# filrg/split_learning

Hardware: AMD Instinct MI355X
Metric: images/sec (whole node) VGG16/CIFAR10 cut=7 (higher is better)
Workload: dtype fp32; 1 GPU; model=VGG16_CIFAR10, global_batch=32, image=3x32x32, cut_layer=7, optimizer=SGD(lr=5e-4, momentum=0.5), control_count=1, mode=serial-recompute, parallelism=split2 x dp1

## Files before the change

### split_learning_amd/ops/build.py

```python

from __future__ import annotations

import os
import subprocess
import sys
import sysconfig
from concurrent.futures import ThreadPoolExecutor

HERE = os.path.dirname(os.path.abspath(__file__))
CSRC = os.path.join(HERE, "csrc")
OUT_SO = os.path.join(HERE, "_sl_kernels.so")
BUILD_DIR = os.path.join(HERE, "_build")

SOURCES = [
    "gemm_f32.hip",
    "conv2d.hip",
    "wino.hip",
    "norm.hip",
    "elementwise.hip",
    "loss.hip",
    "attention.hip",
    "optim.hip",
    "bindings.cpp",
]

ARCH = os.environ.get("PYTORCH_ROCM_ARCH", "gfx950")


def _flags():
    import torch
    import torch.utils.cpp_extension as cpp_ext

    torch_lib = os.path.join(os.path.dirname(torch.__file__), "lib")
    includes = cpp_ext.include_paths(device_type="cuda")
    includes.append(sysconfig.get_paths()["include"])
    abi = int(getattr(torch._C, "_GLIBCXX_USE_CXX11_ABI", True))
    cxxflags = [
        "-O3", "-std=c++17", "-fPIC",
        f"--offload-arch={ARCH}",
        f"-D_GLIBCXX_USE_CXX11_ABI={abi}",
        "-DTORCH_EXTENSION_NAME=_sl_kernels",
        "-DTORCH_API_INCLUDE_EXTENSION_H",
        "-DUSE_ROCM=1",
        "-D__HIP_PLATFORM_AMD__=1",
        "-DHIP_ENABLE_WARP_SYNC_BUILTINS=1",
        "-Wno-deprecated-declarations",
        "-fno-gpu-rdc",
    ] + [f"-I{p}" for p in includes]
    if os.environ.get("SLK_MFMA32"):
        cxxflags.append("-DSLK_MFMA32")
    ldflags = [
        "-shared",
        f"-L{torch_lib}", "-ltorch", "-ltorch_cpu", "-ltorch_python", "-lc10",
        "-ltorch_hip", "-lc10_hip",
        "-L/opt/rocm/lib", "-lamdhip64",
        f"-Wl,-rpath,{torch_lib}",
    ]
    return cxxflags, ldflags


def _run(cmd):
    proc = subprocess.run(cmd, capture_output=True, text=True)
    if proc.returncode != 0:
        raise RuntimeError(
            f"command failed ({proc.returncode}): {' '.join(cmd)}\n"
            f"stdout:\n{proc.stdout[-4000:]}\nstderr:\n{proc.stderr[-8000:]}")
    return proc


def build(verbose: bool = True, force: bool = False) -> str:
    os.makedirs(BUILD_DIR, exist_ok=True)
    hipcc = os.environ.get("HIPCC", "/opt/rocm/bin/hipcc")
    cxxflags, ldflags = _flags()

    objs = []
    jobs = []
    for src in SOURCES:
        sp = os.path.join(CSRC, src)
        op = os.path.join(BUILD_DIR, src.replace("/", "_") + ".o")
        objs.append(op)
        deps = [sp] + [os.path.join(CSRC, h) for h in (
            "common.h", "tile_gemm.h", "torch_util.h", "conv_route.h")]
        if (not force and os.path.exists(op)
                and all(os.path.getmtime(op) >= os.path.getmtime(d) for d in deps)):
            continue
        cmd = [hipcc, "-c", sp, "-o", op] + cxxflags
        if src.endswith(".cpp"):
            cmd.append("-x")
            cmd.append("c++")
        jobs.append(cmd)

    if jobs:
        if verbose:
            print(f"[build] compiling {len(jobs)} TU(s) with {hipcc} for {ARCH}")
        with ThreadPoolExecutor(max_workers=min(8, len(jobs))) as ex:
            list(ex.map(_run, jobs))

    if force or not os.path.exists(OUT_SO) or any(
            os.path.getmtime(o) > os.path.getmtime(OUT_SO) for o in objs):
        if verbose:
# ... 9 lines not shown
```

### split_learning_amd/ops/csrc/bindings.cpp

```cpp
#include <torch/extension.h>

namespace slk {
at::Tensor matmul_f32(const at::Tensor&, const at::Tensor&, bool, bool,
                      c10::optional<at::Tensor>, bool);
at::Tensor linear_fwd(const at::Tensor&, const at::Tensor&, c10::optional<at::Tensor>);
at::Tensor colsum_f32(const at::Tensor&);
at::Tensor conv2d_wino(const at::Tensor&, const at::Tensor&,
                       c10::optional<at::Tensor>, int, bool);
at::Tensor conv2d_wino_bwdw(const at::Tensor&, const at::Tensor&, int);
at::Tensor conv2d_wino_fused(const at::Tensor&, const at::Tensor&,
                             c10::optional<at::Tensor>, int, bool);
at::Tensor conv2d_wino_bwdw_fused(const at::Tensor&, const at::Tensor&, int);
at::Tensor conv2d_fwd(const at::Tensor&, const at::Tensor&, c10::optional<at::Tensor>,
                      int, int);
at::Tensor conv2d_bwd_data(const at::Tensor&, const at::Tensor&, int, int, int, int);
at::Tensor conv2d_bwd_weight(const at::Tensor&, const at::Tensor&, int, int, int, int);
at::Tensor conv2d_bwd_bias(const at::Tensor&);
std::string conv_route(const std::string&, int, int, int, int, int, int, int, int);
std::vector<at::Tensor> bn2d_stats_fused(const at::Tensor&,
                                         c10::optional<at::Tensor>,
                                         c10::optional<at::Tensor>,
                                         c10::optional<at::Tensor>, double, double);
at::Tensor bn2d_fwd(const at::Tensor&, const at::Tensor&, const at::Tensor&,
                    const at::Tensor&, const at::Tensor&, bool);
std::vector<at::Tensor> bn2d_bwd(const at::Tensor&, const at::Tensor&,
                                 const at::Tensor&, const at::Tensor&,
                                 const at::Tensor&, c10::optional<at::Tensor>);
std::vector<at::Tensor> bn2d_bwd_eval(const at::Tensor&, const at::Tensor&,
                                      const at::Tensor&, const at::Tensor&,
                                      const at::Tensor&, c10::optional<at::Tensor>);
std::vector<at::Tensor> bn2d_train_fwd(const at::Tensor&, const at::Tensor&,
                                       const at::Tensor&,
                                       c10::optional<at::Tensor>,
                                       c10::optional<at::Tensor>,
                                       c10::optional<at::Tensor>, double, double,
                                       bool, bool);
std::vector<at::Tensor> bn2d_train_bwd(const at::Tensor&, const at::Tensor&,
                                       const at::Tensor&, const at::Tensor&,
                                       const at::Tensor&, c10::optional<at::Tensor>,
                                       c10::optional<at::Tensor>);
std::vector<at::Tensor> drop_res_ln_fwd(const at::Tensor&, const at::Tensor&,
                                        const at::Tensor&, const at::Tensor&,
                                        double, double, int64_t,
                                        c10::optional<at::Tensor>);
std::vector<at::Tensor> layernorm_fwd(const at::Tensor&, const at::Tensor&,
                                      const at::Tensor&, double);
std::vector<at::Tensor> layernorm_bwd(const at::Tensor&, const at::Tensor&,
                                      const at::Tensor&, const at::Tensor&,
                                      const at::Tensor&);
at::Tensor relu_fwd(const at::Tensor&);
at::Tensor relu_bwd(const at::Tensor&, const at::Tensor&);
at::Tensor gelu_fwd(const at::Tensor&);
at::Tensor gelu_bwd(const at::Tensor&, const at::Tensor&);
at::Tensor tanh_fwd(const at::Tensor&);
at::Tensor tanh_bwd(const at::Tensor&, const at::Tensor&);
std::vector<at::Tensor> dropout_fwd(const at::Tensor&, double, int64_t, int64_t);
std::vector<at::Tensor> dropout_fwd_dev(const at::Tensor&, double, int64_t,
                                        const at::Tensor&);
at::Tensor dropout_bwd(const at::Tensor&, const at::Tensor&, double);
std::vector<at::Tensor> maxpool2x2_fwd(const at::Tensor&);
at::Tensor maxpool2x2_bwd(const at::Tensor&, const at::Tensor&, int, int);
at::Tensor embedding_fwd(const at::Tensor&, const at::Tensor&);
at::Tensor embedding_bwd(const at::Tensor&, const at::Tensor&, int64_t, int64_t);
std::vector<at::Tensor> attn_fwd(const at::Tensor&, const at::Tensor&,
                                 const at::Tensor&, double, double, int64_t,
                                 c10::optional<at::Tensor>);
at::Tensor softmax_fwd(const at::Tensor&);
at::Tensor softmax_bwd(const at::Tensor&, const at::Tensor&);
std::vector<at::Tensor> ce_fwd(const at::Tensor&, const at::Tensor&);
at::Tensor ce_bwd(const at::Tensor&, const at::Tensor&, const at::Tensor&);
void sgd_step(std::vector<at::Tensor>, std::vector<at::Tensor>,
              std::vector<at::Tensor>, double, double, double, bool, bool);
void adamw_step(std::vector<at::Tensor>, std::vector<at::Tensor>,
                std::vector<at::Tensor>, std::vector<at::Tensor>, int64_t, double,
                double, double, double, double, bool);
at::Tensor make_opt_desc(std::vector<at::Tensor>, std::vector<at::Tensor>,
                         std::vector<at::Tensor>, std::vector<at::Tensor>);
void sgd_step_fused(const at::Tensor&, int64_t, int64_t, double, double, double,
                    bool, bool);
void adamw_step_fused(const at::Tensor&, int64_t, int64_t, int64_t, double, double,
                      double, double, double, bool);
}

PYBIND11_MODULE(TORCH_EXTENSION_NAME, m) {
  m.doc() = "split_learning_amd CDNA4 (gfx950) HIP kernels";
  m.def("matmul_f32", &slk::matmul_f32, py::arg("a"), py::arg("b"),
        py::arg("trans_a") = false, py::arg("trans_b") = false,
        py::arg("out") = py::none(), py::arg("accumulate") = false);
  m.def("linear_fwd", &slk::linear_fwd);
  m.def("colsum_f32", &slk::colsum_f32);
  m.def("conv2d_wino", &slk::conv2d_wino, py::arg("x"), py::arg("w"),
        py::arg("bias") = py::none(), py::arg("pad") = 1,
        py::arg("flip") = false);
  m.def("conv2d_wino_bwdw", &slk::conv2d_wino_bwdw, py::arg("gy"),
        py::arg("x"), py::arg("pad") = 1);
  m.def("conv2d_wino_fused", &slk::conv2d_wino_fused, py::arg("x"),
        py::arg("w"), py::arg("bias") = py::none(), py::arg("pad") = 1,
        py::arg("flip") = false);
  m.def("conv2d_wino_bwdw_fused", &slk::conv2d_wino_bwdw_fused, py::arg("gy"),
        py::arg("x"), py::arg("pad") = 1);
  m.def("conv2d_fwd", &slk::conv2d_fwd, py::arg("x"), py::arg("w"),
        py::arg("bias"), py::arg("stride"), py::arg("pad"));
  m.def("conv2d_bwd_data", &slk::conv2d_bwd_data);
  m.def("conv2d_bwd_weight", &slk::conv2d_bwd_weight, py::arg("gy"), py::arg("x"),
        py::arg("kh"), py::arg("kw"), py::arg("stride"), py::arg("pad"));
  m.def("conv2d_bwd_bias", &slk::conv2d_bwd_bias);
  m.def("conv_route", &slk::conv_route, py::arg("op"), py::arg("B"),
        py::arg("Ci"), py::arg("H"), py::arg("W"), py::arg("Co"), py::arg("K"),
        py::arg("stride"), py::arg("pad"));
  m.def("bn2d_stats_fused", &slk::bn2d_stats_fused);
  m.def("bn2d_fwd", &slk::bn2d_fwd);
  m.def("bn2d_bwd", &slk::bn2d_bwd, py::arg("x"), py::arg("gy"),
        py::arg("gamma"), py::arg("mean"), py::arg("invstd"),
        py::arg("relu_y") = py::none());
  m.def("bn2d_bwd_eval", &slk::bn2d_bwd_eval, py::arg("x"), py::arg("gy"),
        py::arg("gamma"), py::arg("mean"), py::arg("invstd"),
        py::arg("relu_y") = py::none());
  m.def("bn2d_train_fwd", &slk::bn2d_train_fwd, py::arg("x"), py::arg("gamma"),
        py::arg("beta"), py::arg("running_mean"), py::arg("running_var"),
        py::arg("num_batches_tracked"), py::arg("momentum"), py::arg("eps"),
        py::arg("relu") = false, py::arg("pool") = false);
  m.def("bn2d_train_bwd", &slk::bn2d_train_bwd, py::arg("x"), py::arg("gy"),
        py::arg("gamma"), py::arg("mean"), py::arg("invstd"),
        py::arg("relu_y") = py::none(), py::arg("idx") = py::none());
  m.def("drop_res_ln_fwd", &slk::drop_res_ln_fwd, py::arg("x"), py::arg("res"),
        py::arg("gamma"), py::arg("beta"), py::arg("eps"), py::arg("p") = 0.0,
        py::arg("seed") = 0, py::arg("offset") = py::none());
  m.def("layernorm_fwd", &slk::layernorm_fwd);
  m.def("layernorm_bwd", &slk::layernorm_bwd);
  m.def("relu_fwd", &slk::relu_fwd);
  m.def("relu_bwd", &slk::relu_bwd);
  m.def("gelu_fwd", &slk::gelu_fwd);
  m.def("gelu_bwd", &slk::gelu_bwd);
  m.def("tanh_fwd", &slk::tanh_fwd);
  m.def("tanh_bwd", &slk::tanh_bwd);
  m.def("dropout_fwd", &slk::dropout_fwd);
  m.def("dropout_fwd_dev", &slk::dropout_fwd_dev);
  m.def("dropout_bwd", &slk::dropout_bwd);
  m.def("maxpool2x2_fwd", &slk::maxpool2x2_fwd);
  m.def("maxpool2x2_bwd", &slk::maxpool2x2_bwd);
  m.def("embedding_fwd", &slk::embedding_fwd);
  m.def("embedding_bwd", &slk::embedding_bwd);
  m.def("attn_fwd", &slk::attn_fwd, py::arg("q"), py::arg("k"), py::arg("v"),
        py::arg("scale"), py::arg("p") = 0.0, py::arg("seed") = 0,
        py::arg("offset") = py::none());
  m.def("softmax_fwd", &slk::softmax_fwd);
  m.def("softmax_bwd", &slk::softmax_bwd);
  m.def("ce_fwd", &slk::ce_fwd);
  m.def("ce_bwd", &slk::ce_bwd);
  m.def("sgd_step", &slk::sgd_step);
  m.def("adamw_step", &slk::adamw_step);
  m.def("make_opt_desc", &slk::make_opt_desc);
  m.def("sgd_step_fused", &slk::sgd_step_fused);
  m.def("adamw_step_fused", &slk::adamw_step_fused);
}
```

### split_learning_amd/ops/csrc/conv2d.hip

```cpp
#include <tuple>

#include "conv_route.h"
#include "tile_gemm.h"
#include "torch_util.h"

namespace slk {

at::Tensor conv2d_wino(const at::Tensor&, const at::Tensor&,
                       c10::optional<at::Tensor>, int, bool);
at::Tensor conv2d_wino_bwdw(const at::Tensor&, const at::Tensor&, int);
at::Tensor conv2d_wino_fused(const at::Tensor&, const at::Tensor&,
                             c10::optional<at::Tensor>, int, bool);
at::Tensor conv2d_wino_bwdw_fused(const at::Tensor&, const at::Tensor&, int);

static int wino_level() {
  static const int v = [] {
    const char* e = std::getenv("SLK_WINO");
    return e ? atoi(e) : 1;
  }();
  return v;
}

struct ConvGeom {
  int B, Ci, H, W, Co, KH, KW, OH, OW, stride, pad;
  FastDiv d_ohow, d_ow, d_hw, d_w, d_khkw, d_kw;
};

template <int CKH, int CKW, int CS>
struct Geo {
  static constexpr bool fixed = CKH > 0;
  __device__ static int kh_kw(const ConvGeom& g) { return fixed ? CKH * CKW : g.KH * g.KW; }
  __device__ static int stride(const ConvGeom& g) { return fixed ? CS : g.stride; }
  __device__ static void dk(const ConvGeom& g, int k, int& c, int& kh, int& kw) {
    if (fixed) {
      c = k / (CKH * CKW);
      const int r = k - c * (CKH * CKW);
      kh = r / CKW;
      kw = r - kh * CKW;
    } else {
      c = g.d_khkw.div(k);
      const int r = g.d_khkw.mod(k, c);
      kh = g.d_kw.div(r);
      kw = g.d_kw.mod(r, kh);
    }
  }
};

__device__ __forceinline__ float sel0(float v, bool keep) { return keep ? v : 0.f; }

template <int CKH, int CKW, int CS>
struct ConvFwdGather {
  using G = Geo<CKH, CKW, CS>;
  const float* w;
  const float* x;
  ConvGeom geo;

  struct KCtx {};
  __device__ KCtx prepK(int) const { return {}; }

  struct ACtx { int off; bool valid; };
  struct BCtx { int boff, ihb, iwb; bool valid; };

  __device__ ACtx prepA(int, int m, bool valid, int) const {
    return {(int)((long)m * (geo.Ci * G::kh_kw(geo))), valid};
  }
  __device__ float loadA(const ACtx& c, const KCtx&, int k, bool kv) const {
    return sel0(w[c.off + k], c.valid & kv);
  }
  __device__ BCtx prepB(int, int n, bool valid, int) const {
    const unsigned b = geo.d_ohow.div(n);
    const unsigned rem = geo.d_ohow.mod(n, b);
    const unsigned oh = geo.d_ow.div(rem);
    const unsigned ow = geo.d_ow.mod(rem, oh);
    return {(int)((long)b * geo.Ci * geo.H * geo.W),
            (int)oh * G::stride(geo) - geo.pad,
            (int)ow * G::stride(geo) - geo.pad, valid};
  }
  __device__ float loadB(const BCtx& c, const KCtx&, int k, bool kv) const {
    int ci, kh, kw;
    G::dk(geo, k, ci, kh, kw);
    const int ih = c.ihb + kh;
    const int iw = c.iwb + kw;
    const bool in = (unsigned)ih < (unsigned)geo.H && (unsigned)iw < (unsigned)geo.W;
    const int ihc = in ? ih : 0;
    const int iwc = in ? iw : 0;
    const float v = x[c.boff + (ci * geo.H + ihc) * geo.W + iwc];
    return sel0(v, c.valid & kv & in);
  }
};

struct ConvFwdStore {
  float* y;
// ... 300 lines not shown
      return conv2d_wino(x, w, bias, pad, false);
    default:
      break;
  }
  auto xc = x.contiguous();
  auto wc = w.contiguous();
  const ConvGeom geo = make_geom(s);
  const float* bp = bias.has_value() ? bias->data_ptr<float>() : nullptr;
  return direct_gemm<ConvFwdGather>(
      geo, geo.Co, geo.B * geo.OH * geo.OW, geo.Ci * geo.KH * geo.KW,
      {geo.B, geo.Co, geo.OH, geo.OW}, x.options(), wc.data_ptr<float>(),
      xc.data_ptr<float>(), [&](float* y, bool accumulate, long slab_stride) {
        return ConvFwdStore{y, bp, geo.Co, geo.OH * geo.OW, geo.d_ohow,
                            accumulate, slab_stride};
      });
}

at::Tensor conv2d_bwd_data(const at::Tensor& gy, const at::Tensor& w, int stride,
                           int pad, int H, int W) {
  TORCH_CHECK(gy.is_cuda() && gy.dim() == 4 && gy.scalar_type() == at::kFloat);
  const ConvShape s = conv_shape(gy.size(0), w.size(1), H, W, w.size(0),
                                 w.size(2), w.size(3), stride, pad);
  TORCH_CHECK(s.OH() == gy.size(2) && s.OW() == gy.size(3),
              "bwd-data geometry mismatch");
  switch (route_bwd_data(s, wino_level())) {
    case ConvRoute::WinoFused:
      return conv2d_wino_fused(gy, w, c10::nullopt, 2 - pad, true);
    case ConvRoute::Wino:
      return conv2d_wino(gy, w, c10::nullopt, 2 - pad, true);
    default:
      break;
  }
  auto gyc = gy.contiguous();
  auto wc = w.contiguous();
  const ConvGeom geo = make_geom(s);
  return direct_gemm<ConvBwdDataGather>(
      geo, geo.Ci, geo.B * H * W, geo.Co * geo.KH * geo.KW,
      {geo.B, geo.Ci, H, W}, gy.options(), wc.data_ptr<float>(),
      gyc.data_ptr<float>(), [&](float* gx, bool accumulate, long slab_stride) {
        return ConvBwdDataStore{gx, geo.Ci, H * W, geo.d_hw, accumulate,
                                slab_stride};
      });
}

at::Tensor conv2d_bwd_weight(const at::Tensor& gy, const at::Tensor& x, int KH,
                             int KW, int stride, int pad) {
  TORCH_CHECK(gy.is_cuda() && x.is_cuda() && gy.scalar_type() == at::kFloat);
  const ConvShape s = conv_shape(x.size(0), x.size(1), x.size(2), x.size(3),
                                 gy.size(1), KH, KW, stride, pad);
  TORCH_CHECK(s.OH() == gy.size(2) && s.OW() == gy.size(3),
              "bwd-weight geometry mismatch");
  switch (route_bwd_weight(s, wino_level())) {
    case ConvRoute::WinoBwdWFused:
      return conv2d_wino_bwdw_fused(gy, x, pad);
    case ConvRoute::WinoBwdW:
      return conv2d_wino_bwdw(gy, x, pad);
    default:
      break;
  }
  auto gyc = gy.contiguous();
  auto xc = x.contiguous();
  const ConvGeom geo = make_geom(s);
  const int N = geo.Ci * KH * KW;
  const bool fast = (geo.OH * geo.OW) % SLK_BK == 0;
  return direct_gemm<ConvBwdWeightGather>(
      geo, geo.Co, N, geo.B * geo.OH * geo.OW, {geo.Co, geo.Ci, KH, KW},
      gy.options(), gyc.data_ptr<float>(), xc.data_ptr<float>(),
      [&](float* gw, bool accumulate, long slab_stride) {
        return AtomicStore{gw, N, accumulate, slab_stride};
      },
      fast);
}

std::string conv_route(const std::string& op, int B, int Ci, int H, int W,
                       int Co, int K, int stride, int pad) {
  const ConvShape s = conv_shape(B, Ci, H, W, Co, K, K, stride, pad);
  if (op == "fwd") return conv_route_name(route_fwd(s, wino_level()));
  if (op == "bwd_data") return conv_route_name(route_bwd_data(s, wino_level()));
  TORCH_CHECK(op == "bwd_weight", "conv_route: op must be fwd, bwd_data or "
              "bwd_weight, got ", op);
  return conv_route_name(route_bwd_weight(s, wino_level()));
}

__global__ void conv_bias_grad_kernel(const float* __restrict__ gy,
                                      float* __restrict__ slab, int B, int C,
                                      int HW) {
  __shared__ float scratch[16];
  const int c = blockIdx.x;
  const int total = B * HW;
  const int per = (total + gridDim.y - 1) / gridDim.y;
  const int lo = blockIdx.y * per;
  const int hi = min(total, lo + per);
  float acc = 0.f;
  for (int i = lo + threadIdx.x; i < hi; i += blockDim.x) {
    const int b = i / HW;
    const int r = i - b * HW;
    acc += gy[((long)b * C + c) * HW + r];
  }
  float total_s = slk_block_sum(acc, scratch);
  if (threadIdx.x == 0) slab[(long)blockIdx.y * C + c] = total_s;
}

__global__ void conv_bias_finalize_kernel(const float* __restrict__ slab,
                                          int chunks, float* __restrict__ gb,
                                          int C) {
  const int c = blockIdx.x * blockDim.x + threadIdx.x;
  if (c >= C) return;
  float s = 0.f;
  for (int k = 0; k < chunks; ++k) s += slab[(long)k * C + c];
  gb[c] = s;
}

at::Tensor conv2d_bwd_bias(const at::Tensor& gy) {
  auto gyc = gy.contiguous();
  const int B = gy.size(0), C = gy.size(1), HW = gy.size(2) * gy.size(3);
  auto gb = at::empty({C}, gy.options());
  const int chunks = reduce_chunks((long)B * HW);
  auto slab = at::empty({chunks, C}, gy.options());
  auto stream = c10::hip::getCurrentHIPStream().stream();
  hipLaunchKernelGGL(conv_bias_grad_kernel, dim3(C, (uint32_t)chunks), dim3(256),
                     0, stream, gyc.data_ptr<float>(), slab.data_ptr<float>(), B, C,
                     HW);
  hipLaunchKernelGGL(conv_bias_finalize_kernel, dim3(ceil_div(C, 256)), dim3(256),
                     0, stream, slab.data_ptr<float>(), chunks,
                     gb.data_ptr<float>(), C);
  return gb;
}

}
```

### split_learning_amd/ops/csrc/conv_route.h

```cpp
#pragma once

namespace slk {

enum class ConvRoute {
  Direct,
  Wino,
  WinoFused,
  WinoBwdW,
  WinoBwdWFused,
};

inline const char* conv_route_name(ConvRoute r) {
  switch (r) {
    case ConvRoute::Direct: return "direct";
    case ConvRoute::Wino: return "wino";
    case ConvRoute::WinoFused: return "wino_fused";
    case ConvRoute::WinoBwdW: return "wino_bwdw";
    case ConvRoute::WinoBwdWFused: return "wino_bwdw_fused";
  }
  return "?";
}

struct ConvShape {
  int B, Ci, H, W, Co, KH, KW, stride, pad;
  int OH() const { return (H + 2 * pad - KH) / stride + 1; }
  int OW() const { return (W + 2 * pad - KW) / stride + 1; }
  bool is_3x3_s1() const { return KH == 3 && KW == 3 && stride == 1; }
};

inline bool wino_fused_ok(int level, int Cin, int Cout, int T, int OH, int OW) {
  if (level == 0) return false;
  if ((OH | OW) & 1) return false;
  if (Cout % 32 != 0 || T % 32 != 0 || Cin % 8 != 0) return false;
  if (level >= 3) return true;
  return (long)(T / 32) * (Cout / 32) >= 256;
}

inline bool wino_wins(int level, int Ci, int Co, int H, int OH, int OW) {
  if (level == 0) return false;
  if ((OH | OW) & 1) return false;
  if (level >= 2) return true;
  return Ci == Co && (Ci >= 256 || H >= 32);
}

inline bool wino_wins_bwdw(int level, int Ci, int Co, int H, int OH, int OW) {
  if (level == 0) return false;
  if ((OH | OW) & 1) return false;
  if (level >= 2) return true;
  return (Ci == Co && H != 4) || (Ci <= 4 && H >= 32);
}

inline ConvRoute route_fwd(const ConvShape& s, int level) {
  if (s.is_3x3_s1()) {
    const int OH = s.OH(), OW = s.OW();
    const int T = s.B * (OH / 2) * (OW / 2);
    if (wino_fused_ok(level, s.Ci, s.Co, T, OH, OW)) return ConvRoute::WinoFused;
    if (wino_wins(level, s.Ci, s.Co, s.H, OH, OW)) return ConvRoute::Wino;
  }
  return ConvRoute::Direct;
}

inline ConvRoute route_bwd_data(const ConvShape& s, int level) {
  if (s.is_3x3_s1() && s.pad <= 2) {
    const int T = s.B * (s.H / 2) * (s.W / 2);
    if (s.H % 2 == 0 && s.W % 2 == 0) {
      if (wino_fused_ok(level, s.Co, s.Ci, T, s.H, s.W)) return ConvRoute::WinoFused;
      if (level != 0 && s.H >= 4 && s.Ci >= 64 && s.Ci % 32 == 0 &&
          s.Co % 8 == 0 && T % 32 == 0 && (long)(T / 32) * (s.Ci / 32) >= 32) {
        return ConvRoute::WinoFused;
      }
    }
    if (wino_wins(level, s.Co, s.Ci, s.OH(), s.H, s.W)) return ConvRoute::Wino;
  }
  return ConvRoute::Direct;
}

inline ConvRoute route_bwd_weight(const ConvShape& s, int level) {
  const int OH = s.OH(), OW = s.OW();
  if (s.is_3x3_s1() && s.pad <= 2 && OH % 2 == 0 && OW % 2 == 0) {
    if (level != 0 && s.Ci % 32 == 0 && s.Co % 32 == 0) {
      return ConvRoute::WinoBwdWFused;
    }
    if (wino_wins_bwdw(level, s.Ci, s.Co, s.H, OH, OW)) return ConvRoute::WinoBwdW;
  }
  return ConvRoute::Direct;
}

}
```

### split_learning_amd/ops/csrc/wino.hip

```cpp
#include "torch_util.h"

namespace slk {

template <bool FLIP>
__global__ void wino_wt_kernel(const float* __restrict__ w,
                               float* __restrict__ U, int Cw0, int Cw1) {
  const long total = (long)Cw0 * Cw1;
  const long tstride = (long)gridDim.x * blockDim.x;
  for (long e = (long)blockIdx.x * blockDim.x + threadIdx.x; e < 4 * total;
       e += tstride) {
    const int a = (int)(e & 3);
    const long i = e >> 2;
    const int cols = FLIP ? Cw0 : Cw1;
    const int c = (int)(i % cols);
    const int r = (int)(i / cols);
    const int co = FLIP ? c : r;
    const int ci = FLIP ? r : c;
    float t[3];
    #pragma unroll
    for (int b = 0; b < 3; ++b) {
      const float g0 = w[(((long)co * Cw1 + ci) * 3 + (FLIP ? 2 : 0)) * 3 +
                         (FLIP ? 2 - b : b)];
      const float g1 = w[(((long)co * Cw1 + ci) * 3 + 1) * 3 +
                         (FLIP ? 2 - b : b)];
      const float g2 = w[(((long)co * Cw1 + ci) * 3 + (FLIP ? 0 : 2)) * 3 +
                         (FLIP ? 2 - b : b)];
      t[b] = a == 0 ? g0
           : a == 1 ? 0.5f * (g0 + g1 + g2)
           : a == 2 ? 0.5f * (g0 - g1 + g2)
           : g2;
    }
    U[((long)(a * 4 + 0) * total) + i] = t[0];
    U[((long)(a * 4 + 1) * total) + i] = 0.5f * (t[0] + t[1] + t[2]);
    U[((long)(a * 4 + 2) * total) + i] = 0.5f * (t[0] - t[1] + t[2]);
    U[((long)(a * 4 + 3) * total) + i] = t[2];
  }
}

__global__ void wino_in_kernel(const float* __restrict__ x,
                               float* __restrict__ V, int B, int Ci, int H,
                               int W, int tH, int tW, int pad, FastDiv d_T,
                               FastDiv d_thw, FastDiv d_tw) {
  const int T = B * tH * tW;
  const long total = (long)Ci * T;
  const long stride = (long)gridDim.x * blockDim.x;
  for (long i = (long)blockIdx.x * blockDim.x + threadIdx.x; i < total;
       i += stride) {
    const unsigned cc = d_T.div((unsigned)i);
    const unsigned t = d_T.mod((unsigned)i, cc);
    const unsigned b = d_thw.div(t);
    const unsigned rem = d_thw.mod(t, b);
    const unsigned th = d_tw.div(rem);
    const unsigned tw = d_tw.mod(rem, th);
    const int ih0 = (int)th * 2 - pad;
    const int iw0 = (int)tw * 2 - pad;
    const float* xp = x + ((long)b * Ci + cc) * H * W;
    float d[4][4];
    #pragma unroll
    for (int a = 0; a < 4; ++a) {
      const int ih = ih0 + a;
      const bool hv = (unsigned)ih < (unsigned)H;
      #pragma unroll
      for (int bb = 0; bb < 4; ++bb) {
        const int iw = iw0 + bb;
        const bool v = hv && (unsigned)iw < (unsigned)W;
        d[a][bb] = v ? xp[(long)ih * W + iw] : 0.f;
      }
    }
    float u[4][4];
    #pragma unroll
    for (int bb = 0; bb < 4; ++bb) {
      u[0][bb] = d[0][bb] - d[2][bb];
      u[1][bb] = d[1][bb] + d[2][bb];
      u[2][bb] = d[2][bb] - d[1][bb];
      u[3][bb] = d[1][bb] - d[3][bb];
    }
    #pragma unroll
    for (int a = 0; a < 4; ++a) {
      const float v0 = u[a][0] - u[a][2];
      const float v1 = u[a][1] + u[a][2];
      const float v2 = u[a][2] - u[a][1];
      const float v3 = u[a][1] - u[a][3];
      V[((long)(a * 4 + 0) * Ci + cc) * T + t] = v0;
      V[((long)(a * 4 + 1) * Ci + cc) * T + t] = v1;
      V[((long)(a * 4 + 2) * Ci + cc) * T + t] = v2;
      V[((long)(a * 4 + 3) * Ci + cc) * T + t] = v3;
    }
  }
}

__global__ void wino_out_kernel(const float* __restrict__ Mm,
                                float* __restrict__ y,
                                const float* __restrict__ bias, int B, int Co,
                                int OH, int OW, int tH, int tW, FastDiv d_T,
                                FastDiv d_thw, FastDiv d_tw) {
  const int T = B * tH * tW;
  const long total = (long)Co * T;
  const long stride = (long)gridDim.x * blockDim.x;
  for (long i = (long)blockIdx.x * blockDim.x + threadIdx.x; i < total;
       i += stride) {
    const unsigned co = d_T.div((unsigned)i);
    const unsigned t = d_T.mod((unsigned)i, co);
    const unsigned b = d_thw.div(t);
    const unsigned rem = d_thw.mod(t, b);
    const unsigned th = d_tw.div(rem);
    const unsigned tw = d_tw.mod(rem, th);
    float m[4][4];
    #pragma unroll
    for (int f = 0; f < 16; ++f)
      m[f >> 2][f & 3] = Mm[((long)f * Co + co) * T + t];
    float u[2][4];
    #pragma unroll
    for (int bb = 0; bb < 4; ++bb) {
      u[0][bb] = m[0][bb] + m[1][bb] + m[2][bb];
      u[1][bb] = m[1][bb] - m[2][bb] - m[3][bb];
    }
    const float bv = bias != nullptr ? bias[co] : 0.f;
    float* yp = y + ((long)b * Co + co) * OH * OW + (long)th * 2 * OW + tw * 2;
    yp[0] = u[0][0] + u[0][1] + u[0][2] + bv;
    yp[1] = u[0][1] - u[0][2] - u[0][3] + bv;
    yp[OW] = u[1][0] + u[1][1] + u[1][2] + bv;
    yp[OW + 1] = u[1][1] - u[1][2] - u[1][3] + bv;
  }
}

__global__ void wino_gyA_kernel(const float* __restrict__ gy,
                                float* __restrict__ Wg, int B, int Co, int OH,
                                int OW, int tH, int tW, FastDiv d_T,
                                FastDiv d_thw, FastDiv d_tw) {
  const int T = B * tH * tW;
  const long total = (long)Co * T;
  const long stride = (long)gridDim.x * blockDim.x;
  for (long i = (long)blockIdx.x * blockDim.x + threadIdx.x; i < total;
       i += stride) {
    const unsigned co = d_T.div((unsigned)i);
    const unsigned t = d_T.mod((unsigned)i, co);
    const unsigned b = d_thw.div(t);
    const unsigned rem = d_thw.mod(t, b);
    const unsigned th = d_tw.div(rem);
    const unsigned tw = d_tw.mod(rem, th);
    const float* gp = gy + ((long)b * Co + co) * OH * OW
                      + (long)th * 2 * OW + tw * 2;
    const float g00 = gp[0], g01 = gp[1], g10 = gp[OW], g11 = gp[OW + 1];
    float r0c0 = g00, r0c1 = g01;
    float r1c0 = g00 + g10, r1c1 = g01 + g11;
    float r2c0 = g00 - g10, r2c1 = g01 - g11;
    float r3c0 = -g10, r3c1 = -g11;
    #pragma unroll
    for (int a = 0; a < 4; ++a) {
      const float c0 = a == 0 ? r0c0 : a == 1 ? r1c0 : a == 2 ? r2c0 : r3c0;
      const float c1 = a == 0 ? r0c1 : a == 1 ? r1c1 : a == 2 ? r2c1 : r3c1;
      Wg[((long)(a * 4 + 0) * Co + co) * T + t] = c0;
      Wg[((long)(a * 4 + 1) * Co + co) * T + t] = c0 + c1;
      Wg[((long)(a * 4 + 2) * Co + co) * T + t] = c0 - c1;
      Wg[((long)(a * 4 + 3) * Co + co) * T + t] = -c1;
    }
  }
}

__global__ void wino_gw_kernel(const float* __restrict__ dU,
                               float* __restrict__ gw, int Co, int Ci) {
  const long total = (long)Co * Ci;
  const long stride = (long)gridDim.x * blockDim.x;
  for (long i = (long)blockIdx.x * blockDim.x + threadIdx.x; i < total;
       i += stride) {
    float u[4][4];
    #pragma unroll
    for (int f = 0; f < 16; ++f) u[f >> 2][f & 3] = dU[(long)f * total + i];
    float t[3][4];
    #pragma unroll
    for (int b = 0; b < 4; ++b) {
      t[0][b] = u[0][b] + 0.5f * (u[1][b] + u[2][b]);
      t[1][b] = 0.5f * (u[1][b] - u[2][b]);
      t[2][b] = 0.5f * (u[1][b] + u[2][b]) + u[3][b];
    }
    #pragma unroll
    for (int r = 0; r < 3; ++r) {
      gw[i * 9 + r * 3 + 0] = t[r][0] + 0.5f * (t[r][1] + t[r][2]);
      gw[i * 9 + r * 3 + 1] = 0.5f * (t[r][1] - t[r][2]);
      gw[i * 9 + r * 3 + 2] = 0.5f * (t[r][1] + t[r][2]) + t[r][3];
    }
  }
}

at::Tensor matmul_f32(const at::Tensor&, const at::Tensor&, bool, bool,
                      c10::optional<at::Tensor>, bool);

at::Tensor conv2d_wino(const at::Tensor& x, const at::Tensor& w,
                       c10::optional<at::Tensor> bias, int pad, bool flip) {
  TORCH_CHECK(x.is_cuda() && x.dim() == 4 && x.scalar_type() == at::kFloat);
  TORCH_CHECK(w.size(2) == 3 && w.size(3) == 3, "wino: 3x3 only");
  auto xc = x.contiguous();
  auto wc = w.contiguous();
  const int B = x.size(0), H = x.size(2), W = x.size(3);
  const int Co = flip ? w.size(1) : w.size(0);
  const int Ci = flip ? w.size(0) : w.size(1);
  TORCH_CHECK(x.size(1) == Ci, "wino: channel mismatch");
  const int OH = H + 2 * pad - 2, OW = W + 2 * pad - 2;
  TORCH_CHECK(OH % 2 == 0 && OW % 2 == 0, "wino: even output dims only");
  const int tH = OH / 2, tW = OW / 2;
  const int T = B * tH * tW;
  auto stream = c10::hip::getCurrentHIPStream().stream();

  auto U = at::empty({16, Co, Ci}, x.options());
  auto V = at::empty({16, Ci, T}, x.options());
  {
    const long tot = (long)Co * Ci * 4;
    const int grid = (int)std::min<long>((tot + 255) / 256, 4096);
    if (flip) {
      hipLaunchKernelGGL(wino_wt_kernel<true>, dim3(grid), dim3(256), 0,
                         stream, wc.data_ptr<float>(), U.data_ptr<float>(),
                         (int)w.size(0), (int)w.size(1));
    } else {
      hipLaunchKernelGGL(wino_wt_kernel<false>, dim3(grid), dim3(256), 0,
                         stream, wc.data_ptr<float>(), U.data_ptr<float>(),
                         (int)w.size(0), (int)w.size(1));
    }
  }
  {
    FastDiv d_T, d_thw, d_tw;
    d_T.init(T);
    d_thw.init(tH * tW);
    d_tw.init(tW);
    const long tot = (long)Ci * T;
    const int grid = (int)std::min<long>((tot + 255) / 256, 8192);
    hipLaunchKernelGGL(wino_in_kernel, dim3(grid), dim3(256), 0, stream,
                       xc.data_ptr<float>(), V.data_ptr<float>(), B, Ci, H, W,
                       tH, tW, pad, d_T, d_thw, d_tw);
  }
  auto Mm = matmul_f32(U, V, false, false, c10::nullopt, false);
  auto y = at::empty({B, Co, OH, OW}, x.options());
  {
    FastDiv d_T, d_thw, d_tw;
    d_T.init(T);
    d_thw.init(tH * tW);
    d_tw.init(tW);
    const long tot = (long)Co * T;
    const int grid = (int)std::min<long>((tot + 255) / 256, 8192);
    hipLaunchKernelGGL(wino_out_kernel, dim3(grid), dim3(256), 0, stream,
                       Mm.data_ptr<float>(), y.data_ptr<float>(),
                       bias.has_value() ? bias->data_ptr<float>() : nullptr,
                       B, Co, OH, OW, tH, tW, d_T, d_thw, d_tw);
  }
  return y;
}


constexpr int WF_CO = 32;
constexpr int WF_T = 32;
constexpr int WF_CK = 8;
constexpr int WF_KS = 20;
constexpr int WF_RS = 168;
constexpr int WF_OP = 32 * WF_RS;

__device__ __forceinline__ void wino_kstep_mfma(const float* pa,
                                                const float* pb,
                                                f32x4 (&acc)[16]) {
  const f32x4* a0 = reinterpret_cast<const f32x4*>(pa);
  const f32x4* a1 = reinterpret_cast<const f32x4*>(pa + 4 * WF_KS);
  const f32x4* b0 = reinterpret_cast<const f32x4*>(pb);
  const f32x4* b1 = reinterpret_cast<const f32x4*>(pb + 4 * WF_KS);
  f32x4 ra0 = a0[0], rb0 = b0[0], ra1 = a1[0], rb1 = b1[0];
  #pragma unroll
  for (int g = 0; g < 4; ++g) {
    const f32x4 ca0 = ra0, cb0 = rb0, ca1 = ra1, cb1 = rb1;
    if (g < 3) {
      ra0 = a0[g + 1];
      rb0 = b0[g + 1];
      ra1 = a1[g + 1];
      rb1 = b1[g + 1];
    }
    __builtin_amdgcn_sched_barrier(0);
    #pragma unroll
    for (int j = 0; j < 4; ++j)
      acc[g * 4 + j] = __builtin_amdgcn_mfma_f32_16x16x4f32(
          ca0[j], cb0[j], acc[g * 4 + j], 0, 0, 0);
    #pragma unroll
    for (int j = 0; j < 4; ++j)
      acc[g * 4 + j] = __builtin_amdgcn_mfma_f32_16x16x4f32(
          ca1[j], cb1[j], acc[g * 4 + j], 0, 0, 0);
  }
}

template <bool FLIP>
__global__ __launch_bounds__(256, 3) void wino_fused_kernel(
    const float* __restrict__ x, const float* __restrict__ w,
    const float* __restrict__ bias, float* __restrict__ y, int B, int Ci,
    int H, int W, int Co, int OH, int OW, int tH, int tW, int pad,
    int ci_per, int CW, FastDiv d_thw, FastDiv d_tw) {
  const int ci_begin = blockIdx.z * ci_per;
  const int ci_end = min(Ci, ci_begin + ci_per);
  __shared__ __attribute__((aligned(16))) float Ul[WF_OP];
  __shared__ __attribute__((aligned(16))) float Vl[WF_OP];

  const int T = B * tH * tW;
  const int co0 = blockIdx.y * WF_CO;
  const int t0 = blockIdx.x * WF_T;

  const int tid = threadIdx.x;
  const int lane = tid & 63;
  const int wid = tid >> 6;
  const int wco = (wid >> 1) * 16;
  const int wt = (wid & 1) * 16;
  const int frag_r = lane >> 4;
  const int frag_c = lane & 15;

  f32x4 acc[16];
  #pragma unroll
  for (int f = 0; f < 16; ++f) acc[f] = f32x4{};

  const int v_ci = tid >> 5;
// ... 399 lines not shown
```

Baseline: 14520 images/sec.

## Add direct 2x2-image tile1 conv path and fuse winograd weight/input transforms

Adds a specialized direct-convolution kernel for 3x3 convs on 2x2 spatial inputs (a single Winograd tile), keeping weights in registers and reducing over input channels via shared memory and split slabs. It is gated behind the SLK_WINO_TILE1 environment variable, so it is off by default. Separately, the Winograd weight-transform and input-transform kernels are merged into one launch that partitions blocks between the two jobs, removing one kernel launch per winograd conv call. The fused launch runs by default and trades a branch per block for the saved launch.

```diff
diff --git a/split_learning_amd/ops/build.py b/split_learning_amd/ops/build.py
--- a/split_learning_amd/ops/build.py
+++ b/split_learning_amd/ops/build.py
@@ -16,6 +16,7 @@
     "gemm_f32.hip",
     "conv2d.hip",
     "wino.hip",
+    "wino_tile1.hip",
     "norm.hip",
     "elementwise.hip",
     "loss.hip",
diff --git a/split_learning_amd/ops/csrc/bindings.cpp b/split_learning_amd/ops/csrc/bindings.cpp
--- a/split_learning_amd/ops/csrc/bindings.cpp
+++ b/split_learning_amd/ops/csrc/bindings.cpp
@@ -6,7 +6,9 @@
 at::Tensor linear_fwd(const at::Tensor&, const at::Tensor&, c10::optional<at::Tensor>);
 at::Tensor colsum_f32(const at::Tensor&);
 at::Tensor conv2d_wino(const at::Tensor&, const at::Tensor&,
-                       c10::optional<at::Tensor>, int, bool);
+                       c10::optional<at::Tensor>, int, bool, const std::string&);
+at::Tensor conv2d_wino_tile1(const at::Tensor&, const at::Tensor&,
+                             c10::optional<at::Tensor>, int, bool);
 at::Tensor conv2d_wino_bwdw(const at::Tensor&, const at::Tensor&, int);
 at::Tensor conv2d_wino_fused(const at::Tensor&, const at::Tensor&,
                              c10::optional<at::Tensor>, int, bool);
@@ -17,6 +19,9 @@
 at::Tensor conv2d_bwd_weight(const at::Tensor&, const at::Tensor&, int, int, int, int);
 at::Tensor conv2d_bwd_bias(const at::Tensor&);
 std::string conv_route(const std::string&, int, int, int, int, int, int, int, int);
+std::string conv_wino_form(const std::string&, int, int, int, int, int, int, int,
+                           int);
+bool conv_wino_tile1_enabled();
 std::vector<at::Tensor> bn2d_stats_fused(const at::Tensor&,
                                          c10::optional<at::Tensor>,
                                          c10::optional<at::Tensor>,
@@ -91,6 +96,9 @@
   m.def("colsum_f32", &slk::colsum_f32);
   m.def("conv2d_wino", &slk::conv2d_wino, py::arg("x"), py::arg("w"),
         py::arg("bias") = py::none(), py::arg("pad") = 1,
+        py::arg("flip") = false, py::arg("form") = "auto");
+  m.def("conv2d_wino_tile1", &slk::conv2d_wino_tile1, py::arg("x"),
+        py::arg("w"), py::arg("bias") = py::none(), py::arg("pad") = 1,
         py::arg("flip") = false);
   m.def("conv2d_wino_bwdw", &slk::conv2d_wino_bwdw, py::arg("gy"),
         py::arg("x"), py::arg("pad") = 1);
@@ -108,6 +116,10 @@
   m.def("conv_route", &slk::conv_route, py::arg("op"), py::arg("B"),
         py::arg("Ci"), py::arg("H"), py::arg("W"), py::arg("Co"), py::arg("K"),
         py::arg("stride"), py::arg("pad"));
+  m.def("conv_wino_form", &slk::conv_wino_form, py::arg("op"), py::arg("B"),
+        py::arg("Ci"), py::arg("H"), py::arg("W"), py::arg("Co"), py::arg("K"),
+        py::arg("stride"), py::arg("pad"));
+  m.def("conv_wino_tile1_enabled", &slk::conv_wino_tile1_enabled);
   m.def("bn2d_stats_fused", &slk::bn2d_stats_fused);
   m.def("bn2d_fwd", &slk::bn2d_fwd);
   m.def("bn2d_bwd", &slk::bn2d_bwd, py::arg("x"), py::arg("gy"),
diff --git a/split_learning_amd/ops/csrc/conv2d.hip b/split_learning_amd/ops/csrc/conv2d.hip
--- a/split_learning_amd/ops/csrc/conv2d.hip
+++ b/split_learning_amd/ops/csrc/conv2d.hip
@@ -6,8 +6,11 @@
 
 namespace slk {
 
+bool wino_tile1_enabled();
+
 at::Tensor conv2d_wino(const at::Tensor&, const at::Tensor&,
-                       c10::optional<at::Tensor>, int, bool);
+                       c10::optional<at::Tensor>, int, bool,
+                       const std::string& form = "auto");
 at::Tensor conv2d_wino_bwdw(const at::Tensor&, const at::Tensor&, int);
 at::Tensor conv2d_wino_fused(const at::Tensor&, const at::Tensor&,
                              c10::optional<at::Tensor>, int, bool);
@@ -474,6 +477,16 @@
   return conv_route_name(route_bwd_weight(s, wino_level()));
 }
 
+std::string conv_wino_form(const std::string& op, int B, int Ci, int H, int W,
+                           int Co, int K, int stride, int pad) {
+  TORCH_CHECK(op == "fwd" || op == "bwd_data",
+              "conv_wino_form: op must be fwd or bwd_data, got ", op);
+  const ConvShape s = conv_shape(B, Ci, H, W, Co, K, K, stride, pad);
+  return wino_form_name(wino_form(s, op == "bwd_data", wino_level()));
+}
+
+bool conv_wino_tile1_enabled() { return wino_tile1_enabled(); }
+
 __global__ void conv_bias_grad_kernel(const float* __restrict__ gy,
                                       float* __restrict__ slab, int B, int C,
                                       int HW) {
diff --git a/split_learning_amd/ops/csrc/conv_route.h b/split_learning_amd/ops/csrc/conv_route.h
--- a/split_learning_amd/ops/csrc/conv_route.h
+++ b/split_learning_amd/ops/csrc/conv_route.h
@@ -75,6 +75,22 @@
   return ConvRoute::Direct;
 }
 
+enum class WinoForm { Pipeline, Tile1 };
+
+inline const char* wino_form_name(WinoForm f) {
+  return f == WinoForm::Tile1 ? "tile1" : "pipeline";
+}
+
+inline WinoForm wino_form(const ConvShape& s, bool flip, int level) {
+  (void)flip;
+  if (level == 0 || !s.is_3x3_s1()) return WinoForm::Pipeline;
+  if (s.H != 2 || s.W != 2 || s.pad != 1) return WinoForm::Pipeline;
+  if (s.Ci < 4 || s.Co < 4 || s.Ci % 4 != 0 || s.Co % 4 != 0) {
+    return WinoForm::Pipeline;
+  }
+  return WinoForm::Tile1;
+}
+
 inline ConvRoute route_bwd_weight(const ConvShape& s, int level) {
   const int OH = s.OH(), OW = s.OW();
   if (s.is_3x3_s1() && s.pad <= 2 && OH % 2 == 0 && OW % 2 == 0) {
diff --git a/split_learning_amd/ops/csrc/wino.hip b/split_learning_amd/ops/csrc/wino.hip
--- a/split_learning_amd/ops/csrc/wino.hip
+++ b/split_learning_amd/ops/csrc/wino.hip
@@ -1,14 +1,17 @@
+#include <string>
+
+#include "conv_route.h"
 #include "torch_util.h"
 
 namespace slk {
 
 template <bool FLIP>
-__global__ void wino_wt_kernel(const float* __restrict__ w,
-                               float* __restrict__ U, int Cw0, int Cw1) {
+__device__ __forceinline__ void wino_wt_body(const float* __restrict__ w,
+                                             float* __restrict__ U, int Cw0,
+                                             int Cw1, long first,
+                                             long tstride) {
   const long total = (long)Cw0 * Cw1;
-  const long tstride = (long)gridDim.x * blockDim.x;
-  for (long e = (long)blockIdx.x * blockDim.x + threadIdx.x; e < 4 * total;
-       e += tstride) {
+  for (long e = first; e < 4 * total; e += tstride) {
     const int a = (int)(e & 3);
     const long i = e >> 2;
     const int cols = FLIP ? Cw0 : Cw1;
@@ -37,15 +40,13 @@
   }
 }
 
-__global__ void wino_in_kernel(const float* __restrict__ x,
-                               float* __restrict__ V, int B, int Ci, int H,
-                               int W, int tH, int tW, int pad, FastDiv d_T,
-                               FastDiv d_thw, FastDiv d_tw) {
+__device__ __forceinline__ void wino_in_body(
+    const float* __restrict__ x, float* __restrict__ V, int B, int Ci, int H,
+    int W, int tH, int tW, int pad, FastDiv d_T, FastDiv d_thw, FastDiv d_tw,
+    long first, long stride) {
   const int T = B * tH * tW;
   const long total = (long)Ci * T;
-  const long stride = (long)gridDim.x * blockDim.x;
-  for (long i = (long)blockIdx.x * blockDim.x + threadIdx.x; i < total;
-       i += stride) {
+  for (long i = first; i < total; i += stride) {
     const unsigned cc = d_T.div((unsigned)i);
     const unsigned t = d_T.mod((unsigned)i, cc);
     const unsigned b = d_thw.div(t);
@@ -86,6 +87,34 @@
       V[((long)(a * 4 + 2) * Ci + cc) * T + t] = v2;
       V[((long)(a * 4 + 3) * Ci + cc) * T + t] = v3;
     }
+  }
+}
+
+__global__ void wino_in_kernel(const float* __restrict__ x,
+                               float* __restrict__ V, int B, int Ci, int H,
+                               int W, int tH, int tW, int pad, FastDiv d_T,
+                               FastDiv d_thw, FastDiv d_tw) {
+  wino_in_body(x, V, B, Ci, H, W, tH, tW, pad, d_T, d_thw, d_tw,
+               (long)blockIdx.x * blockDim.x + threadIdx.x,
+               (long)gridDim.x * blockDim.x);
+}
+
+template <bool FLIP>
+__global__ void wino_wt_in_kernel(const float* __restrict__ w,
+                                  float* __restrict__ U, int Cw0, int Cw1,
+                                  int wt_blocks, const float* __restrict__ x,
+                                  float* __restrict__ V, int B, int Ci, int H,
+                                  int W, int tH, int tW, int pad, FastDiv d_T,
+                                  FastDiv d_thw, FastDiv d_tw) {
+  if ((int)blockIdx.x < wt_blocks) {
+    wino_wt_body<FLIP>(w, U, Cw0, Cw1,
+                       (long)blockIdx.x * blockDim.x + threadIdx.x,
+                       (long)wt_blocks * blockDim.x);
+  } else {
+    const int in_blocks = (int)gridDim.x - wt_blocks;
+    wino_in_body(x, V, B, Ci, H, W, tH, tW, pad, d_T, d_thw, d_tw,
+                 (long)((int)blockIdx.x - wt_blocks) * blockDim.x + threadIdx.x,
+                 (long)in_blocks * blockDim.x);
   }
 }
 
@@ -186,10 +215,24 @@
 at::Tensor matmul_f32(const at::Tensor&, const at::Tensor&, bool, bool,
                       c10::optional<at::Tensor>, bool);
 
+at::Tensor conv2d_wino_tile1(const at::Tensor&, const at::Tensor&,
+                             c10::optional<at::Tensor>, int, bool);
+bool wino_tile1_enabled();
+ConvShape wino_call_shape(const at::Tensor&, const at::Tensor&, int, bool);
+
 at::Tensor conv2d_wino(const at::Tensor& x, const at::Tensor& w,
-                       c10::optional<at::Tensor> bias, int pad, bool flip) {
+                       c10::optional<at::Tensor> bias, int pad, bool flip,
+                       const std::string& form) {
   TORCH_CHECK(x.is_cuda() && x.dim() == 4 && x.scalar_type() == at::kFloat);
   TORCH_CHECK(w.size(2) == 3 && w.size(3) == 3, "wino: 3x3 only");
+  TORCH_CHECK(form == "auto" || form == "pipeline" || form == "tile1",
+              "wino: form must be auto, pipeline or tile1");
+  if (form == "tile1") return conv2d_wino_tile1(x, w, bias, pad, flip);
+  if (form == "auto" && wino_tile1_enabled() &&
+      x.size(1) == (flip ? w.size(0) : w.size(1)) &&
+      wino_form(wino_call_shape(x, w, pad, flip), flip, 1) == WinoForm::Tile1) {
+    return conv2d_wino_tile1(x, w, bias, pad, flip);
+  }
   auto xc = x.contiguous();
   auto wc = w.contiguous();
   const int B = x.size(0), H = x.size(2), W = x.size(3);
@@ -205,28 +248,27 @@
   auto U = at::empty({16, Co, Ci}, x.options());
   auto V = at::empty({16, Ci, T}, x.options());
   {
-    const long tot = (long)Co * Ci * 4;
-    const int grid = (int)std::min<long>((tot + 255) / 256, 4096);
-    if (flip) {
-      hipLaunchKernelGGL(wino_wt_kernel<true>, dim3(grid), dim3(256), 0,
-                         stream, wc.data_ptr<float>(), U.data_ptr<float>(),
-                         (int)w.size(0), (int)w.size(1));
-    } else {
-      hipLaunchKernelGGL(wino_wt_kernel<false>, dim3(grid), dim3(256), 0,
-                         stream, wc.data_ptr<float>(), U.data_ptr<float>(),
-                         (int)w.size(0), (int)w.size(1));
-    }
-  }
-  {
+    const long wtot = (long)Co * Ci * 4;
+    const int wt_blocks = (int)std::min<long>((wtot + 255) / 256, 4096);
+    const long itot = (long)Ci * T;
+    const int in_blocks = (int)std::min<long>((itot + 255) / 256, 8192);
     FastDiv d_T, d_thw, d_tw;
     d_T.init(T);
     d_thw.init(tH * tW);
     d_tw.init(tW);
-    const long tot = (long)Ci * T;
-    const int grid = (int)std::min<long>((tot + 255) / 256, 8192);
-    hipLaunchKernelGGL(wino_in_kernel, dim3(grid), dim3(256), 0, stream,
-                       xc.data_ptr<float>(), V.data_ptr<float>(), B, Ci, H, W,
-                       tH, tW, pad, d_T, d_thw, d_tw);
+    if (flip) {
+      hipLaunchKernelGGL(wino_wt_in_kernel<true>, dim3(wt_blocks + in_blocks),
+                         dim3(256), 0, stream, wc.data_ptr<float>(),
+                         U.data_ptr<float>(), (int)w.size(0), (int)w.size(1),
+                         wt_blocks, xc.data_ptr<float>(), V.data_ptr<float>(),
+                         B, Ci, H, W, tH, tW, pad, d_T, d_thw, d_tw);
+    } else {
+      hipLaunchKernelGGL(wino_wt_in_kernel<false>, dim3(wt_blocks + in_blocks),
+                         dim3(256), 0, stream, wc.data_ptr<float>(),
+                         U.data_ptr<float>(), (int)w.size(0), (int)w.size(1),
+                         wt_blocks, xc.data_ptr<float>(), V.data_ptr<float>(),
+                         B, Ci, H, W, tH, tW, pad, d_T, d_thw, d_tw);
+    }
   }
   auto Mm = matmul_f32(U, V, false, false, c10::nullopt, false);
   auto y = at::empty({B, Co, OH, OW}, x.options());
diff --git a/split_learning_amd/ops/csrc/wino_tile1.hip b/split_learning_amd/ops/csrc/wino_tile1.hip
--- /dev/null
+++ b/split_learning_amd/ops/csrc/wino_tile1.hip
@@ -0,0 +1,246 @@
+#include "conv_route.h"
+#include "torch_util.h"
+
+namespace slk {
+
+typedef float f32x2 __attribute__((ext_vector_type(2)));
+
+constexpr int T1_BT = 32;
+constexpr int T1_SB = 16;
+constexpr int T1_THREADS = 256;
+
+template <bool FLIP>
+struct T1Cfg {
+  static constexpr int OCL = FLIP ? 16 : 8;
+  static constexpr int LG = 64 / OCL;
+  static constexpr int P = 4 * LG;
+  static constexpr int RCB = 4 * P;
+  static constexpr int E4 = T1_SB * OCL;
+  static constexpr int PSTRIDE = E4 + 8;
+  static constexpr int XS4 = T1_BT * RCB;
+  static constexpr int SMEM4 = XS4 + P * PSTRIDE;
+};
+
+template <bool FLIP>
+__device__ constexpr int t1_tap(int i, int o) {
+  return FLIP ? 4 + 3 * ((o >> 1) - (i >> 1)) + ((o & 1) - (i & 1))
+              : 4 + 3 * ((i >> 1) - (o >> 1)) + ((i & 1) - (o & 1));
+}
+
+template <bool FLIP>
+__global__ __launch_bounds__(T1_THREADS) void wino_tile1_kernel(
+    const float* __restrict__ x,
+    const float* __restrict__ w,
+    const float* __restrict__ bias,
+    float* __restrict__ out,
+    int B, int Ci, int Co) {
+  using C = T1Cfg<FLIP>;
+  __shared__ float4 sm[C::SMEM4];
+  float4* red = sm + C::XS4;
+  const int tid = threadIdx.x;
+  const int lane = tid & 63, wave = tid >> 6;
+  const int ocl = lane % C::OCL, g = lane / C::OCL;
+  const int p = wave * C::LG + g;
+  const int s = blockIdx.y;
+  const int Coc = FLIP ? Ci : Co;
+  const int Crc = FLIP ? Co : Ci;
+  const int oc = blockIdx.x * C::OCL + ocl;
+  const int rc0 = s * C::RCB + p * 4;
+  const float4* x4 = reinterpret_cast<const float4*>(x);
+  float2* out2 = reinterpret_cast<float2*>(out);
+
+  float wr[4][9];
+  if (oc < Coc && rc0 < Crc) {
+    if (!FLIP) {
+      const float4* wp =
+          reinterpret_cast<const float4*>(w + ((long)oc * Ci + rc0) * 9);
+      float4 t4[9];
+      #pragma unroll
+      for (int j = 0; j < 9; ++j) t4[j] = wp[j];
+      #pragma unroll
+      for (int j = 0; j < 9; ++j) {
+        (&wr[0][0])[j * 4 + 0] = t4[j].x;
+        (&wr[0][0])[j * 4 + 1] = t4[j].y;
+        (&wr[0][0])[j * 4 + 2] = t4[j].z;
+        (&wr[0][0])[j * 4 + 3] = t4[j].w;
+      }
+    } else {
+      #pragma unroll
+      for (int q = 0; q < 4; ++q) {
+        const float* wp = w + ((long)(rc0 + q) * Ci + oc) * 9;
+        #pragma unroll
+        for (int t = 0; t < 9; ++t) wr[q][t] = wp[t];
+      }
+    }
+  } else {
+    #pragma unroll
+    for (int q = 0; q < 4; ++q)
+      #pragma unroll
+      for (int t = 0; t < 9; ++t) wr[q][t] = 0.f;
+  }
+
+  for (int bt0 = 0; bt0 < B; bt0 += T1_BT) {
+    {
+      constexpr int N = C::XS4 / 2 / T1_THREADS;
+      float4 v0[N], v1[N];
+      #pragma unroll
+      for (int k = 0; k < N; ++k) {
+        const int idx = tid + k * T1_THREADS;
+        const int b = bt0 + 2 * (idx / C::RCB);
+        const int rc = s * C::RCB + idx % C::RCB;
+        const bool ok0 = b < B && rc < Crc, ok1 = b + 1 < B && rc < Crc;
+        v0[k] = x4[ok0 ? (long)b * Crc + rc : 0];
+        v1[k] = x4[ok1 ? (long)(b + 1) * Crc + rc : 0];
+      }
+      #pragma unroll
+      for (int k = 0; k < N; ++k) {
+        const int idx = tid + k * T1_THREADS;
+        const int bp = idx / C::RCB, rcl = idx % C::RCB;
+        const int b = bt0 + 2 * bp;
+        const int rc = s * C::RCB + rcl;
+        const bool ok0 = b < B && rc < Crc, ok1 = b + 1 < B && rc < Crc;
+        const int grp = rcl >> 2, q = rcl & 3;
+        const int pos = ((grp / C::LG) * 4 + q) * C::LG + grp % C::LG;
+        const float4 z = make_float4(0.f, 0.f, 0.f, 0.f);
+        const float4 a0 = ok0 ? v0[k] : z, a1 = ok1 ? v1[k] : z;
+        sm[(bp * C::RCB + pos) * 2 + 0] = make_float4(a0.x, a1.x, a0.y, a1.y);
+        sm[(bp * C::RCB + pos) * 2 + 1] = make_float4(a0.z, a1.z, a0.w, a1.w);
+      }
+    }
+    __syncthreads();
+
+    #pragma unroll 1
+    for (int sb0 = 0; sb0 < T1_BT && bt0 + sb0 < B; sb0 += T1_SB) {
+      f32x2 acc[T1_SB / 2][4];
+      #pragma unroll
+      for (int bp = 0; bp < T1_SB / 2; ++bp) {
+        float4 a4[4][2];
+        #pragma unroll
+        for (int q = 0; q < 4; ++q)
+          #pragma unroll
+          for (int h = 0; h < 2; ++h)
+            a4[q][h] = sm[((sb0 / 2 + bp) * C::RCB + (wave * 4 + q) * C::LG + g) * 2 + h];
+        #pragma unroll
+        for (int o = 0; o < 4; ++o) acc[bp][o] = f32x2{0.f, 0.f};
+        #pragma unroll
+        for (int q = 0; q < 4; ++q) {
+          const f32x2 a[4] = {{a4[q][0].x, a4[q][0].y}, {a4[q][0].z, a4[q][0].w},
+                              {a4[q][1].x, a4[q][1].y}, {a4[q][1].z, a4[q][1].w}};
+          #pragma unroll
+          for (int i = 0; i < 4; ++i)
+            #pragma unroll
+            for (int o = 0; o < 4; ++o) {
+              const float wv = wr[q][t1_tap<FLIP>(i, o)];
+              acc[bp][o] = __builtin_elementwise_fma(a[i], f32x2{wv, wv}, acc[bp][o]);
+            }
+        }
+      }
+      #pragma unroll
+      for (int bp = 0; bp < T1_SB / 2; ++bp)
+        #pragma unroll
+        for (int h = 0; h < 2; ++h)
+          red[p * C::PSTRIDE + (bp * C::OCL + ocl) * 2 + h] =
+              make_float4(acc[bp][2 * h][0], acc[bp][2 * h][1],
+                          acc[bp][2 * h + 1][0], acc[bp][2 * h + 1][1]);
+      __syncthreads();
+
+      for (int e = tid; e < C::E4; e += T1_THREADS) {
+        float4 r = red[e];
+        #pragma unroll 8
+        for (int pp = 1; pp < C::P; ++pp) {
+          const float4 t = red[pp * C::PSTRIDE + e];
+          r.x += t.x; r.y += t.y; r.z += t.z; r.w += t.w;
+        }
+        const int h = e & 1;
+        const int o_c = blockIdx.x * C::OCL + (e >> 1) % C::OCL;
+        const int b = bt0 + sb0 + 2 * ((e >> 1) / C::OCL);
+        if (o_c < Coc) {
+          if (bias != nullptr && s == 0) {
+            const float bv = bias[o_c];
+            r.x += bv; r.y += bv; r.z += bv; r.w += bv;
+          }
+          if (b < B)
+            out2[(((long)s * B + b) * Coc + o_c) * 2 + h] = make_float2(r.x, r.z);
+          if (b + 1 < B)
+            out2[(((long)s * B + b + 1) * Coc + o_c) * 2 + h] = make_float2(r.y, r.w);
+        }
+      }
+      __syncthreads();
+    }
+  }
+}
+
+bool wino_tile1_enabled() {
+  static const bool v = [] {
+    const char* e = std::getenv("SLK_WINO_TILE1");
+    return e != nullptr && atoi(e) != 0;
+  }();
+  return v;
+}
+
+ConvShape wino_call_shape(const at::Tensor& x, const at::Tensor& w, int pad,
+                          bool flip) {
+  const int B = x.size(0), H = x.size(2), W = x.size(3);
+  if (!flip) {
+    return ConvShape{B, (int)w.size(1), H, W, (int)w.size(0), 3, 3, 1, pad};
+  }
+  const int pf = 2 - pad;
+  return ConvShape{B, (int)w.size(1), H + 2 - 2 * pf, W + 2 - 2 * pf,
+                   (int)w.size(0), 3, 3, 1, pf};
+}
+
+static at::Tensor aligned16(const at::Tensor& t) {
+  auto c = t.contiguous();
+  if (reinterpret_cast<uintptr_t>(c.data_ptr<float>()) % 16 != 0) c = c.clone();
+  return c;
+}
+
+at::Tensor conv2d_wino_tile1(const at::Tensor& x, const at::Tensor& w,
+                             c10::optional<at::Tensor> bias, int pad,
+                             bool flip) {
+  TORCH_CHECK(x.is_cuda() && x.dim() == 4 && x.scalar_type() == at::kFloat);
+  TORCH_CHECK(w.is_cuda() && w.dim() == 4 && w.scalar_type() == at::kFloat);
+  TORCH_CHECK(w.size(2) == 3 && w.size(3) == 3, "wino tile1: 3x3 only");
+  const int Co = w.size(0), Ci = w.size(1);
+  TORCH_CHECK(x.size(1) == (flip ? Co : Ci), "wino tile1: channel mismatch");
+  TORCH_CHECK(wino_form(wino_call_shape(x, w, pad, flip), flip, 1) ==
+                  WinoForm::Tile1,
+              "wino tile1: needs a 2x2 image at pad 1 and Ci, Co multiples "
+              "of 4");
+  const int B = x.size(0);
+  const int Coc = flip ? Ci : Co, Crc = flip ? Co : Ci;
+  auto xc = aligned16(x);
+  auto wc = aligned16(w);
+  const float* bp = nullptr;
+  at::Tensor bc;
+  if (bias.has_value()) {
+    TORCH_CHECK(bias->numel() == Coc, "wino tile1: bias size");
+    bc = bias->contiguous();
+    bp = bc.data_ptr<float>();
+  }
+  auto stream = c10::hip::getCurrentHIPStream().stream();
+  auto y = at::empty({B, Coc, 2, 2}, x.options());
+  const int ocl = flip ? T1Cfg<true>::OCL : T1Cfg<false>::OCL;
+  const int rcb = flip ? T1Cfg<true>::RCB : T1Cfg<false>::RCB;
+  const int splits = (Crc + rcb - 1) / rcb;
+  const dim3 grid((Coc + ocl - 1) / ocl, splits);
+  at::Tensor slab;
+  float* op = y.data_ptr<float>();
+  if (splits > 1) {
+    slab = at::empty({splits, B, Coc, 2, 2}, x.options());
+    op = slab.data_ptr<float>();
+  }
+  if (flip) {
+    hipLaunchKernelGGL(wino_tile1_kernel<true>, grid, dim3(T1_THREADS), 0,
+                       stream, xc.data_ptr<float>(), wc.data_ptr<float>(), bp,
+                       op, B, Ci, Co);
+  } else {
+    hipLaunchKernelGGL(wino_tile1_kernel<false>, grid, dim3(T1_THREADS), 0,
+                       stream, xc.data_ptr<float>(), wc.data_ptr<float>(), bp,
+                       op, B, Ci, Co);
+  }
+  if (splits > 1) slab_reduce(op, splits, y.data_ptr<float>(), y.numel(), stream);
+  return y;
+}
+
+}
```

New measurement: 14600 images/sec (median of 6 runs). Within noise of the previous version (+0.5%).
